# Luonic/semi-supervised_semantic_segmentation

Hardware: AMD Instinct MI355X
Metric: images/sec (UNet-R50 512x512 bs=16/GPU, mean-teacher + CowMix semi-supervised training step) (higher is better)
Workload: dtype bf16; 1 GPU; C2: UNet(ResNet-50 encoder, max_width=128, ConvT up) 512x512, semi-supervised mean-teacher + CowMix step (BCE sup loss w=0.5, consistency w=10, SGD m=0.9); global_batch=16, per_gpu_batch=16, image_size=512, parallelism=dp1

## Files before the change

include/ssseg.h:

```cpp
#ifndef SSSEG_H
#define SSSEG_H
#include <stdint.h>
#include <stddef.h>

#ifdef __cplusplus
extern "C" {
#endif

typedef struct ihipStream_t* ssseg_stream_t;

enum { SSSEG_F32 = 0, SSSEG_BF16 = 1, SSSEG_F16 = 2, SSSEG_F64 = 3  };
enum { SSSEG_OK = 0, SSSEG_EINVAL = -1, SSSEG_EUNSUPPORTED = -2, SSSEG_EWORKSPACE = -3, SSSEG_ECOMM = -4 };

const char* ssseg_version(void);


size_t ssseg_cowmix_workspace_bytes(int64_t B, int64_t H, int64_t W);

int ssseg_cowmix_mask(const float* noise, const float* sigma, const float* p, int64_t B, int64_t H,
                      int64_t W, float* mask_out, float* field_out, float* thr_out, void* workspace,
                      size_t workspace_bytes, ssseg_stream_t stream);

int ssseg_normal_f32(float* out, int64_t n, uint64_t seed, uint64_t offset, ssseg_stream_t stream);

// ... 285 lines not shown
  int32_t relu;
  float slope;
  double* stats;
  int64_t stats_ld;
  int64_t* stats_rows_host;
} ssseg_conv_epilogue;
int ssseg_conv_igemm_epi(const void* x, const void* w, void* y, const ssseg_conv_desc* desc_host, int dt, int dt_out,
                         const ssseg_conv_epilogue* epi, void* ws, size_t ws_bytes, ssseg_stream_t stream);
int ssseg_conv_igemm_epi_actmask(const void* x, const void* w, void* y, const ssseg_conv_desc* desc_host, int dt,
                                 int dt_out, const ssseg_conv_epilogue* epi, int act, float slope, void* ws,
                                 size_t ws_bytes, ssseg_stream_t stream);
int ssseg_conv_igemm_epi_join(const void* x, const void* w, void* y, const ssseg_conv_desc* desc_host, int dt,
                              int dt_out, const ssseg_conv_epilogue* epi, const void* mask, int64_t ldm, void* ws,
                              size_t ws_bytes, ssseg_stream_t stream);
typedef struct {
  const void* x2;
  int64_t c1;
  int64_t ldx2;
} ssseg_vcat;

int ssseg_conv_igemm_epi_vcat(const void* x, const ssseg_vcat* vc, const void* w, void* y,
                              const ssseg_conv_desc* desc_host, int dt, int dt_out, const ssseg_conv_epilogue* epi,
                              void* ws, size_t ws_bytes, ssseg_stream_t stream);
int ssseg_conv_igemm_epi_vsplit(const void* x, const void* w, void* y, const ssseg_vcat* ysplit,
                                const ssseg_conv_desc* desc_host, int dt, int dt_out, const ssseg_conv_epilogue* epi,
                                void* ws, size_t ws_bytes, ssseg_stream_t stream);
int ssseg_conv_igemm_phases(const void* x, void* y, const ssseg_conv_desc* desc_host, int dt, int dt_out,
                            const ssseg_conv_epilogue* epi, int64_t nphase, const int64_t* phase_geom,
                            const void* const* w, ssseg_stream_t stream);
size_t ssseg_conv_igemm_phases_workspace_bytes(const ssseg_conv_desc* desc_host, int64_t nphase, int dt);
int ssseg_conv_igemm_phases_ws(const void* x, void* y, const ssseg_conv_desc* desc_host, int dt, int dt_out,
                               const ssseg_conv_epilogue* epi, int64_t nphase, const int64_t* phase_geom,
                               const void* const* w, void* ws, size_t ws_bytes, ssseg_stream_t stream);

int ssseg_conv_stem_epi(const void* x, const void* w4, void* y, const ssseg_conv_desc* desc_host, int dt,
                        const ssseg_conv_epilogue* epi, ssseg_stream_t stream);
size_t ssseg_conv_igemm_workspace_bytes(const ssseg_conv_desc* desc_host, int dt);

int ssseg_set_knob(int id, int value);

int64_t ssseg_tune_table_export(unsigned long long* keys_host, int32_t* variants_host, int64_t cap);
int ssseg_tune_table_import(const unsigned long long* keys_host, const int32_t* variants_host, int64_t n,
                            int overwrite);

size_t ssseg_conv_wgrad_workspace_bytes(const ssseg_conv_desc* desc_host, int dt);
int ssseg_conv_wgrad(const void* x, const void* dy, float* dw, const ssseg_conv_desc* desc_host, int dt, int64_t c_real,
                     int64_t k_real, int layout, int accumulate, void* ws, size_t ws_bytes, ssseg_stream_t stream);

size_t ssseg_conv_wgrad2_workspace_bytes(const ssseg_conv_desc* desc_host, int64_t n2, int dt);
int ssseg_conv_wgrad2(const void* x, const void* dy, const void* x2, const void* dy2, int64_t n2, float* dw,
                      const ssseg_conv_desc* desc_host, int dt, int64_t c_real, int64_t k_real, int layout,
                      int accumulate, void* ws, size_t ws_bytes, ssseg_stream_t stream);

int ssseg_conv_wgrad_vcat(const void* x, const ssseg_vcat* vc, const void* dy, float* dw,
                          const ssseg_conv_desc* desc_host, int dt, int64_t c_real, int64_t k_real, int layout,
                          int accumulate, void* ws, size_t ws_bytes, ssseg_stream_t stream);
int ssseg_conv_wgrad2_vcat(const void* x, const ssseg_vcat* vc, const void* dy, const void* x2, const ssseg_vcat* vc2,
                           const void* dy2, int64_t n2, float* dw, const ssseg_conv_desc* desc_host, int dt,
                           int64_t c_real, int64_t k_real, int layout, int accumulate, void* ws, size_t ws_bytes,
                           ssseg_stream_t stream);

int ssseg_weight_pack(const float* src, void* dst, int64_t Kd, int64_t Kr, int64_t Cd, int64_t Rs, int64_t Ss,
                      int64_t Cp, int layout, int64_t r0, int64_t rstep, int64_t Rn, int64_t s0, int64_t sstep,
                      int64_t Sn, int dt, ssseg_stream_t stream);

typedef struct ssseg_pack_desc {
// ... 239 lines not shown
```

semi-supervised_semantic_segmentation_amd/csrc/conv.hip:

```cpp
#include <mutex>
#include <algorithm>
#include <unordered_map>
#include <vector>

#include "conv_kernels.h"

int g_knobs[17] = {0, -1, 0, 0, 0, 1, 0, 0, 0, 0, 100, 0, 0, 0, 0, 0, 0};
thread_local int t_dsplit = 1;

constexpr long long TICKET_POOL = 1 << 20;
__device__ unsigned g_ticket_pool[TICKET_POOL];

unsigned* ticket_slots(long long n) {
  static unsigned* const base = [] {
    void* p = nullptr;
    return hipGetSymbolAddress(&p, HIP_SYMBOL(g_ticket_pool)) == hipSuccess ? (unsigned*)p : nullptr;
  }();
  static std::mutex mu;
  static long long next = 0;
  if (!base || n <= 0 || n > TICKET_POOL / 16) return nullptr;
  std::lock_guard<std::mutex> lk(mu);
  if (next + n > TICKET_POOL) next = 0;
  unsigned* p = base + next;
  next += n;
// ... 184 lines not shown
static int heuristic_variant(const ConvGeom& g) {
  auto tiles = [&](int bm, int bn) { return ((g.M + bm - 1) / bm) * ((g.K + bn - 1) / bn); };
  if (g.KK <= 128) return 0;
  if (g.C % 64) return 5;
  if (g.K > 64) return tiles(256, 128) >= 128 ? 6 : (tiles(128, 128) >= 256 ? 8 : 5);
  return tiles(64, 64) < 512 ? 10 : 0;
}

static int dsplit_plan(const ConvGeom& g, int nph) {
  const int kn = g_knobs[14];
  if (kn < 0 || g.KK == 0) return 1;
  const int nk = (g.C % 64 == 0) ? g.R * g.S * (g.C / 64) : (g.KK + 63) / 64;
  if (kn > 0) return (kn == 2 || kn == 4 || kn == 8) && nk >= kn ? kn : 1;
  const long long t = (long long)nph * ((g.M + 127) / 128) * ((g.K + 63) / 64);
  if (t < 512 && nk >= 64) return (t < 128 && nk >= 128) ? 4 : 2;
  if (t < 256 && nk >= 8) {
    int S = 8;
    while (S > 1 && (t * S > 512 || nk < 4 * S)) S >>= 1;
    return S;
  }
  return 1;
}

template <typename T, typename TO>
int run_variant(int v, const void* x, const void* w, void* y, const ConvGeom& g, const Epi<TO>& ep, unsigned xb,
                unsigned wb, hipStream_t s, float* ws, const PhaseTab* ph = nullptr, const void* x2 = nullptr,
                unsigned x2b = 0) {
  t_pw_rows = -1;
  if (t_dsplit > 1 && (v == 0 || v >= 24)) return -1;
  if constexpr (sizeof(TO) == 2) {
    if (v != 0) return launch_glds_cfg<TO>(v, x, w, y, g, ep, xb, wb, s, ws, ph, x2, x2b);
  }
  if (x2) return -1;
  ws = nullptr;
  if (ph && ph->n > 1) {
    int bm = 0;
    long long rows = 0;
    for (int p = 0; p < ph->n; ++p) {
      ConvGeom gp = g;
      gp.py = ph->py[p];
      gp.px = ph->px[p];
      gp.ooy = ph->ooy[p];
      gp.oox = ph->oox[p];
      Epi<TO> ep2 = ep;
      if (ep.stats) ep2.stats = ep.stats + rows * 2 * ep.sld;
      bm = dispatch_regstaged<T, TO>(x, ph->w[p], y, gp, ep2, ws, s);
      if (bm <= 0) return bm;
      rows += (g.M + bm - 1) / bm;
    }
    return bm;
  }
  return dispatch_regstaged<T, TO>(x, w, y, g, ep, ws, s);
}

template <typename T, typename TO>
int tune_variant(const void* x, const void* w, void* y, const ConvGeom& g, const Epi<TO>& ep, unsigned xb,
                 unsigned wb, hipStream_t s, float* ws, const PhaseTab* ph, const void* x2, unsigned x2b,
                 bool* cache_it) {
  hipStreamCaptureStatus cap = hipStreamCaptureStatusNone;
  const int heur = x2 && heuristic_variant(g) == 0 ? 5 : heuristic_variant(g);
  *cache_it = true;
  if (hipStreamIsCapturing(s, &cap) != hipSuccess || cap != hipStreamCaptureStatusNone) {
    *cache_it = false;
    return heur;
  }
  hipEvent_t e0, e1;
// ... 84 lines not shown
        v = (g.C > g.ldx || S > 1) ? 14 : 0;
        if (x2 && v == 0) return -1;
      } else if ((g.C > g.ldx || S > 1) && (g_knobs[4] == 24 || g_knobs[4] == 28)) {
        v = 14;
      }
      int r = run_variant<T, TO>(v, x, w, y, g, ep, (unsigned)xb, (unsigned)wb, s, wsv, ph, x2, (unsigned)x2b);
      if (r == -1 && S > 1 && g_knobs[4] != 0)
        return run_variant<T, TO>(14, x, w, y, g, ep, (unsigned)xb, (unsigned)wb, s, wsv, ph, x2, (unsigned)x2b);
      if (r == -1 && g_knobs[4] != 0 && !x2 && g.C % 64 && g.C <= g.ldx)
        return run_variant<T, TO>(0, x, w, y, g, ep, 0, 0, s, nullptr, ph);
      if (r == -1 && ep.zmask) {
        int hv = heuristic_variant(g);
        if ((g.C > g.ldx || S > 1) && (hv == 0 || hv >= 24)) hv = 14;
        return run_variant<T, TO>(hv, x, w, y, g, ep, (unsigned)xb, (unsigned)wb, s, S > 1 ? wsv : nullptr, ph);
      }
      if (r == -1 && g_knobs[4] >= 24 && g_knobs[4] <= 28) {
        const int hv = x2 && heuristic_variant(g) == 0 ? 5 : heuristic_variant(g);
        return run_variant<T, TO>(hv, x, w, y, g, ep, (unsigned)xb, (unsigned)wb, s, nullptr, ph, x2, (unsigned)x2b);
      }
      if (r == -1 && g_knobs[4] == 0 && v != 0) {
        int hv = x2 && heuristic_variant(g) == 0 ? 5 : heuristic_variant(g);
        if ((g.C > g.ldx || S > 1) && (hv == 0 || hv >= 24)) hv = 14;
        if (hv != v)
          return run_variant<T, TO>(hv, x, w, y, g, ep, (unsigned)xb, (unsigned)wb, s, wsv, ph, x2, (unsigned)x2b);
      }
      return r;
    }
  }
  if (x2) return -1;
  if (g.C > g.ldx) return SSSEG_EUNSUPPORTED;
  return run_variant<T, TO>(0, x, w, y, g, ep, 0, 0, s, nullptr, ph);
}

bool geom_ok(const ConvGeom& g, int dt) {
  const int vec = (dt == SSSEG_F32 ? 4 : 8);
  if (g.C % vec || g.ldx % vec || g.ldw % vec) return false;
  if (g.N < 1 || g.OH < 1 || g.OW < 1 || g.K < 1 || g.C < 1) return false;
  if (g.M >= 0x7fffffffLL) return false;
  if (g.R < 0 || g.S < 0) return false;
  return true;
}

}

extern "C" int ssseg_set_knob(int id, int value) {
  if (id < 0 || id >= 17) return SSSEG_EINVAL;
  if (id == 6 && value) {
    std::lock_guard<std::mutex> lk(g_variant_mu);
    g_variant.clear();
    return 0;
  }
  g_knobs[id] = value;
  return 0;
}

extern "C" int64_t ssseg_tune_table_export(unsigned long long* keys_host, int32_t* variants_host, int64_t cap) {
  std::lock_guard<std::mutex> lk(g_variant_mu);
  if (cap > 0 && (!keys_host || !variants_host)) return SSSEG_EINVAL;
  std::vector<std::pair<unsigned long long, int>> rows(g_variant.begin(), g_variant.end());
  std::sort(rows.begin(), rows.end());
  const int64_t n = (int64_t)rows.size();
  for (int64_t i = 0; i < n && i < cap; ++i) {
    keys_host[i] = rows[i].first;
    variants_host[i] = rows[i].second;
  }
  return n;
// ... 250 lines not shown
    const int64_t* q = phase_geom + 4 * p;
    for (int k = 0; k < 4; ++k)
      if (q[k] < -0x40000000LL || q[k] > 0x40000000LL) return SSSEG_EINVAL;
    if (!w[p]) return SSSEG_EINVAL;
    ph.py[p] = (int)q[0];
    ph.px[p] = (int)q[1];
    ph.ooy[p] = (int)q[2];
    ph.oox[p] = (int)q[3];
    ph.w[p] = w[p];
  }
  g.py = ph.py[0];
  g.px = ph.px[0];
  g.ooy = ph.ooy[0];
  g.oox = ph.oox[0];
  hipStream_t s = (hipStream_t)stream;
  const size_t need = igemm_ws_bytes(g, dt, (int)nphase);
  float* wsf = (need > 0 && ws && ws_bytes >= need) ? (float*)ws : nullptr;
  int bm;
  if (dt == SSSEG_BF16) {
    const Epi<bf16_t> eb{e.scale, e.shift, (const bf16_t*)e.residual, (int)e.ldr, e.relu, (bf16_t*)e.aux, e.slope,
                         e.stats, (int)e.stats_ld};
    bm = dispatch_igemm<bf16_t, bf16_t>(x, w[0], y, g, eb, wsf, s, &ph);
  } else {
    const Epi<f16_t> eh{e.scale, e.shift, (const f16_t*)e.residual, (int)e.ldr, e.relu, (f16_t*)e.aux, e.slope,
                        e.stats, (int)e.stats_ld};
    bm = dispatch_igemm<f16_t, f16_t>(x, w[0], y, g, eh, wsf, s, &ph);
  }
  if (bm <= 0) return SSSEG_EUNSUPPORTED;
  if (e.stats_rows_host && e.stats) *e.stats_rows_host = nphase * ((g.M + bm - 1) / bm);
  SSSEG_LAUNCH_CHECK();
  return 0;
}

extern "C" int ssseg_conv_igemm_phases(const void* x, void* y, const ssseg_conv_desc* d, int dt, int dt_out,
                                       const ssseg_conv_epilogue* epi, int64_t nphase, const int64_t* phase_geom,
                                       const void* const* w, ssseg_stream_t stream) {
  return ssseg_conv_igemm_phases_ws(x, y, d, dt, dt_out, epi, nphase, phase_geom, w, nullptr, 0, stream);
}
```

semi-supervised_semantic_segmentation_amd/csrc/conv_kernels.h:

```cpp
#pragma once
#include <algorithm>
#include <type_traits>

#include "common.h"

typedef __bf16 bf16x8 __attribute__((ext_vector_type(8)));
typedef _Float16 f16x8 __attribute__((ext_vector_type(8)));

typedef short s16x4 __attribute__((ext_vector_type(4)));
typedef float f32x4 __attribute__((ext_vector_type(4)));

template <typename T16> struct M16;
template <> struct M16<bf16_t> {
  __device__ __forceinline__ static f32x4 mma(const bf16x8& a, const bf16x8& b, const f32x4& c) {
    return __builtin_amdgcn_mfma_f32_16x16x32_bf16(a, b, c, 0, 0, 0);
  }
};
template <> struct M16<f16_t> {
  __device__ __forceinline__ static f32x4 mma(const bf16x8& a, const bf16x8& b, const f32x4& c) {
    return __builtin_amdgcn_mfma_f32_16x16x32_f16(__builtin_bit_cast(f16x8, a), __builtin_bit_cast(f16x8, b), c, 0, 0,
                                                  0);
  }
};
typedef __attribute__((address_space(3))) s16x4 lds_s16x4;
// ... 161 lines not shown
    for (int e = 0; e < V; ++e) {
      s1[e] += __shfl_xor(s1[e], o, 64);
      s2[e] += __shfl_xor(s2[e], o, 64);
    }
  }
  lds_barrier();
  double* red = (double*)smem;
  const int w = threadIdx.x >> 6;
  if (holder)
#pragma unroll
    for (int e = 0; e < V; ++e) {
      red[(w * BN + cofs + e) * 2] = (double)s1[e];
      red[(w * BN + cofs + e) * 2 + 1] = (double)s2[e];
    }
  lds_barrier();
  for (int c = threadIdx.x; c < BN; c += NW * 64) {
    const int n = n0 + c;
    if (n >= sld || (dbg & 4)) continue;
    double a = 0.0, b = 0.0;
#pragma unroll
    for (int k = 0; k < NW; ++k) {
      a += red[(k * BN + c) * 2];
      b += red[(k * BN + c) * 2 + 1];
    }
    stats[(mtile * 2) * sld + n] = a;
    stats[(mtile * 2 + 1) * sld + n] = b;
  }
}

struct PhaseTab {
  int n;
  int py[4], px[4], ooy[4], oox[4];
  const void* w[4];
};

template <typename TO> struct Load4;
template <> struct Load4<float> {
  __device__ __forceinline__ static void ld(const float* p, float (&v)[4]) {
    const float4 q = *(const float4*)p;
    v[0] = q.x; v[1] = q.y; v[2] = q.z; v[3] = q.w;
  }
};
template <> struct Load4<f16_t> {
  __device__ __forceinline__ static void ld(const f16_t* p, float (&v)[4]) { H16::ld4(p, v); }
};
template <> struct Load4<bf16_t> {
  __device__ __forceinline__ static void ld(const bf16_t* p, float (&v)[4]) {
    const uint2 q = *(const uint2*)p;
    v[0] = __uint_as_float(q.x << 16); v[1] = __uint_as_float(q.x & 0xffff0000u);
    v[2] = __uint_as_float(q.y << 16); v[3] = __uint_as_float(q.y & 0xffff0000u);
  }
};

template <typename TO, int FM, int FN, bool ST = false, bool JOIN = false>
__device__ __forceinline__ void store_tile(const f32x4 (&acc)[FN][FM], long long mb, int nb, int lane,
                                           const ConvGeom& g, TO* __restrict__ y, const Epi<TO>& ep,
                                           double (*st1)[4] = nullptr, double (*st2)[4] = nullptr) {
  long long op[FM];
#pragma unroll
  for (int j = 0; j < FM; ++j) {
    const long long m = mb + j * 16 + (lane & 15);
    op[j] = -1;
    if (m < g.M) {
      op[j] = out_pixel(g, (int)m);
    }
  }
// ... 715 lines not shown
                                                                float* __restrict__ ws, unsigned* tix, PhaseTab ph,
                                                                const TO* __restrict__ x2, unsigned x2bytes) {
  constexpr int ROW = 128;
  constexpr bool VC = KM == 1, GK = KM == 2;
  constexpr int STAGE = (BM + BN) * ROW;
  constexpr int AI = BM / 8 / NW;
  constexpr int BI = BN / 8 / NW;
  constexpr int NL = AI + BI;
  constexpr int WTM = BM / WM, WTN = BN / WN, FM = WTM / 16, FN = WTN / 16;
  static_assert(WM * WN == NW && FM >= 1 && FN >= 1 && AI >= 1 && BI >= 1 && NS >= 1 && NS <= 4, "tile");
  constexpr int EPI = BM * (BN * 4 + 16);
  constexpr int SMEM = (NS == 1 && EPI > STAGE) ? EPI : NS * STAGE;
  __shared__ __attribute__((aligned(1024))) char smem[SMEM];

  const int t = threadIdx.x, lane = t & 63, wave = __builtin_amdgcn_readfirstlane(t >> 6);
  const int wm = wave / WN, wn = wave % WN;
  const int nnt = (g.K + BN - 1) / BN;
  const int lsp = 31 - __builtin_clz((unsigned)splits);
  const int bid = xcd_tile(blockIdx.x, gridDim.x);
  const int tile = bid >> lsp, slice = bid & (splits - 1);
  static_assert(BN == 64 || BN == 128 || BN == 256, "n-tile divisor magic");
  const int mt_ = fdiv(tile, BN == 64 ? g.mn64 : (BN == 128 ? g.mn128 : g.mn256),
                       BN == 64 ? g.sn64 : (BN == 128 ? g.sn128 : g.sn256));
  const long long m0 = (long long)mt_ * BM;
  const int n0 = (tile - mt_ * nnt) * BN;
  if (ph.n > 1) {
    const int p = blockIdx.y;
    g.py = ph.py[p];
    g.px = ph.px[p];
    g.ooy = ph.ooy[p];
    g.oox = ph.oox[p];
    w = (const TO*)ph.w[p];
    if (ep.stats) ep.stats += (long long)p * ((g.M + BM - 1) / BM) * 2 * ep.sld;
  }
  const int RS = g.R * g.S;
  const int cpt = g.C >> 6;
  const int nk_all = GK ? (g.KK + 63) >> 6 : RS * cpt;
  int kt0 = 0, nk = nk_all;
  if (splits > 1) {
    const int kper = (nk_all + splits - 1) / splits;
    kt0 = min(nk_all, slice * kper);
    nk = min(nk_all, kt0 + kper) - kt0;
  }
  const __amdgpu_buffer_rsrc_t xr = __builtin_amdgcn_make_buffer_rsrc((void*)x, (short)0, (int)xbytes, 0x00020000);
  const __amdgpu_buffer_rsrc_t wr = __builtin_amdgcn_make_buffer_rsrc((void*)w, (short)0, (int)wbytes, 0x00020000);
  __amdgpu_buffer_rsrc_t xr2 = xr;
  if constexpr (VC) xr2 = __builtin_amdgcn_make_buffer_rsrc((void*)x2, (short)0, (int)x2bytes, 0x00020000);

  const int c_even = (lane & 7) ^ (lane >> 4);
  int a_off[AI], a_iy[AI], a_ix[AI];
  int a_pix[VC ? AI : 1];
  int a_k[GK ? AI : 1];
#pragma unroll
  for (int ii = 0; ii < AI; ++ii) {
    const int inst = wave * AI + ii;
    const int ch = c_even ^ ((inst & 1) * 4);
    const long long m = m0 + 8 * inst + (lane >> 3);
    int pix = 0;
    if (m < g.M && g.aident) {
      a_iy[ii] = 0;
      a_ix[ii] = 0;
      pix = (int)m;
    } else if (m < g.M) {
      int img, oy, ox;
      decode_m(g, (int)m, img, oy, ox);
      a_iy[ii] = oy * g.sy + g.py;
// ... 376 lines not shown
```

semi-supervised_semantic_segmentation_amd/ssseg/native.py:

```python
import ctypes
import os
import re

import torch

_HERE = os.path.dirname(os.path.abspath(__file__))
LIB_PATH = os.environ.get('SSSEG_LIB_PATH') or os.path.join(_HERE, 'libssseg.so')
HEADER = os.path.join(_HERE, '..', '..', 'include', 'ssseg.h')

F32, BF16, F16, F64 = 0, 1, 2, 3
SSSEG_SUM, SSSEG_AVG = 0, 1
_ERRS = {-1: 'SSSEG_EINVAL', -2: 'SSSEG_EUNSUPPORTED', -3: 'SSSEG_EWORKSPACE', -4: 'SSSEG_ECOMM'}

vp, i64, i32, f32, f64, sz, u64 = (ctypes.c_void_p, ctypes.c_int64, ctypes.c_int, ctypes.c_float, ctypes.c_double,
                                   ctypes.c_size_t, ctypes.c_uint64)
I64P = ctypes.POINTER(ctypes.c_int64)

class CatPart(ctypes.Structure):
    _fields_ = [('src', vp), ('dst', vp), ('add', vp), ('ld', i64), ('c', i64)]


def cat_parts(rows):
    return (CatPart * len(rows))(*[CatPart(*r) for r in rows])

# ... 77 lines not shown
    'ssseg_dice_prob_bwd': (i32, [vp, i64, i64, i32, f32, vp, vp, vp, sz, vp]),
    'ssseg_binary_entropy_fwd': (i32, [vp, i64, vp, vp, sz, vp]),
    'ssseg_binary_entropy_bwd': (i32, [vp, i64, vp, vp, vp]),
    'ssseg_entropy_fwd': (i32, [vp, i64, i64, i64, vp, vp, sz, vp]),
    'ssseg_entropy_bwd': (i32, [vp, i64, i64, i64, vp, vp, vp]),
    'ssseg_bce_logits_red_fwd': (i32, [vp, vp, i64, i32, vp, vp, sz, vp]),
    'ssseg_bce_logits_red_bwd': (i32, [vp, vp, i64, i32, vp, vp, vp]),
    'ssseg_smooth_labels': (i32, [vp, vp, i64, f32, f32, vp]),
    'ssseg_uncertainty_workspace_bytes': (sz, [i64, i64, i64]),
    'ssseg_uncertainty_scores': (i32, [vp, i64, i64, i64, vp, vp, sz, vp]),
    'ssseg_kmeans_workspace_bytes': (sz, [i64, i64, i64]),
    'ssseg_kmeans_seed': (i32, [vp, i64, i64, i64, vp, vp, vp, vp, sz, vp]),
    'ssseg_kmeans_fit': (i32, [vp, i64, i64, i64, f64, i64, vp, vp, vp, vp, vp, sz, vp]),
    'ssseg_prob_onehot': (i32, [vp, i64, i64, vp, vp, vp]),
    'ssseg_seg_metrics': (i32, [vp, I64P, i64, i64, vp, I64P, i64, i64, i64, vp, vp, vp, vp]),
    'ssseg_seg_metrics_mc': (i32, [vp, I64P, i64, i64, vp, I64P, i32, i32, i64, i64, i64, i64, i64, vp, vp, vp, vp,
                                   vp]),
    'ssseg_prob_onehot_mc': (i32, [vp, i64, i64, i64, i32, vp, vp, vp]),
    'ssseg_ema_update': (i32, [vp, vp, i64, f64, vp]),
    'ssseg_scale_f32': (i32, [vp, i64, f32, vp]),
    'ssseg_axpby': (i32, [vp, f32, vp, f32, vp, i64, vp]),
    'ssseg_sigmoid_fwd': (i32, [vp, vp, i64, vp]),
    'ssseg_sigmoid_bwd': (i32, [vp, vp, vp, i64, vp]),
    'ssseg_sqnorm_accum': (i32, [vp, i64, vp, vp, sz, vp]),
    'ssseg_sgd_step': (i32, [vp, vp, vp, vp, i64, f32, f32, f32, f32, vp, i32, vp, vp]),
    'ssseg_optim_prepare': (i32, [vp, i32, f64, f64, f64, f64, f64, i64, f64, vp, vp, vp]),
    'ssseg_optim_step': (i32, [vp, vp, vp, vp, vp, vp, vp, i64, i32, i32, f64, f64, f64, f64, f64, f64, vp, vp]),
    'ssseg_amp_update': (i32, [vp, vp, f32, f32, i32, vp]),
    'ssseg_scale_by': (i32, [vp, vp, vp, i64, vp]),
    'ssseg_conv_igemm': (i32, [vp, vp, vp, vp, i32, i32, vp, i32, vp, sz, vp]),
    'ssseg_conv_igemm_phases': (i32, [vp, vp, vp, i32, i32, vp, i64, vp, vp, vp]),
    'ssseg_conv_igemm_phases_ws': (i32, [vp, vp, vp, i32, i32, vp, i64, vp, vp, vp, sz, vp]),
    'ssseg_conv_igemm_phases_workspace_bytes': (sz, [vp, i64, i32]),
    'ssseg_conv_stem_epi': (i32, [vp, vp, vp, vp, i32, vp, vp]),
    'ssseg_conv_igemm_epi': (i32, [vp, vp, vp, vp, i32, i32, vp, vp, sz, vp]),
    'ssseg_conv_igemm_epi_actmask': (i32, [vp, vp, vp, vp, i32, i32, vp, i32, f32, vp, sz, vp]),
    'ssseg_conv_igemm_epi_join': (i32, [vp, vp, vp, vp, i32, i32, vp, vp, i64, vp, sz, vp]),
    'ssseg_weight_pack_batch': (i32, [vp, i64, i32, vp]),
    'ssseg_param_step': (i32, [vp, vp, vp, vp, vp, i64, vp, f32, f32, f32, f32, vp, i32, vp, f64, i32, vp]),
    'ssseg_dwconv_fwd': (i32, [vp, vp, vp, vp, i32, vp, vp]),
    'ssseg_dwconv_dgrad': (i32, [vp, vp, vp, vp, i32, vp]),
    'ssseg_dwconv_wgrad_workspace_bytes': (sz, [vp, i32]),
    'ssseg_dwconv_wgrad': (i32, [vp, vp, vp, vp, i32, i64, i32, vp, sz, vp]),
    'ssseg_conv_igemm_workspace_bytes': (sz, [vp, i32]),
    'ssseg_set_knob': (i32, [i32, i32]),
    'ssseg_tune_table_export': (i64, [vp, vp, i64]),
    'ssseg_tune_table_import': (i32, [vp, vp, i64, i32]),
    'ssseg_conv_wgrad_workspace_bytes': (sz, [vp, i32]),
    'ssseg_conv_wgrad': (i32, [vp, vp, vp, vp, i32, i64, i64, i32, i32, vp, sz, vp]),
    'ssseg_conv_wgrad2_workspace_bytes': (sz, [vp, i64, i32]),
    'ssseg_conv_wgrad2': (i32, [vp, vp, vp, vp, i64, vp, vp, i32, i64, i64, i32, i32, vp, sz, vp]),
    'ssseg_conv_igemm_epi_vcat': (i32, [vp, vp, vp, vp, vp, i32, i32, vp, vp, sz, vp]),
    'ssseg_conv_igemm_epi_vsplit': (i32, [vp, vp, vp, vp, vp, i32, i32, vp, vp, sz, vp]),
    'ssseg_conv_wgrad_vcat': (i32, [vp, vp, vp, vp, vp, i32, i64, i64, i32, i32, vp, sz, vp]),
    'ssseg_conv_wgrad2_vcat': (i32, [vp, vp, vp, vp, vp, vp, i64, vp, vp, i32, i64, i64, i32, i32, vp, sz, vp]),
    'ssseg_weight_pack': (i32, [vp, vp, i64, i64, i64, i64, i64, i64, i32, i64, i64, i64, i64, i64, i64, i32, vp]),
    'ssseg_bn_workspace_bytes': (sz, [i64]),
    'ssseg_bn_stats': (i32, [vp, i64, i64, i64, i32, vp, vp, sz, vp]),
    'ssseg_bn_partials_finalize': (i32, [vp, i64, i64, vp, f64, f32, f32, vp, vp, vp, vp, vp, vp]),
    'ssseg_bn_gstat_finalize': (i32, [vp, i64, i64, vp, vp, vp, vp, vp, vp, vp, vp, vp]),
    'ssseg_bn_gstat_finalize_x': (i32, [vp, i64, i64, vp, vp, vp, vp, vp, i64, i64, i32, vp, vp, vp, vp, vp]),
    'ssseg_channel_sum_grad': (i32, [vp, i64, i64, i64, i32, vp, vp, vp, sz, vp]),
    'ssseg_bn_finalize': (i32, [vp, i64, f64, f32, f32, vp, vp, vp, vp, vp, vp]),
    'ssseg_bn_eval_params': (i32, [vp, vp, f32, i64, vp, vp, vp]),
    'ssseg_bn_fold': (i32, [vp, vp, vp, vp, vp, f32, i64, i64, vp, vp, vp, vp, vp]),
    'ssseg_bn_fold_batch': (i32, [vp, i64, vp]),
# ... 166 lines not shown
```

semi-supervised_semantic_segmentation_amd/ssseg/nn.py:

```python
import contextlib
import ctypes
import os

import torch
import torch.distributed as dist
import torch.nn as nn

from . import comm as _comm
from . import native as N

_CFG = {'act_mask': os.environ.get('SSSEG_ACT_MASK', '1') != '0',
        'grad_join': True, 'stem': os.environ.get('SSSEG_STEM', '1') != '0', 'phases': True, 'eval_bwd_y': True, 'dtype': torch.bfloat16, 'sync_bn': True,
        'fuse_stats': True, 'vcat': os.environ.get('SSSEG_VCAT', '1') != '0',
        'vpad': os.environ.get('SSSEG_VPAD', '1') != '0',
        'bn_gstat': os.environ.get('SSSEG_BN_GSTAT', '1') != '0',
        'bn_join': os.environ.get('SSSEG_BN_JOIN', '1') != '0'}


_QUANT = [None]


def set_bn_grad_stats(on):
    _CFG['bn_gstat'] = bool(on)


def set_bn_join(on):
    _CFG['bn_join'] = bool(on)


def _bn_join_on():
    return _CFG['bn_join'] and _CFG['bn_gstat'] and _CFG['act_mask']


def set_virtual_concat(on):
    _CFG['vcat'] = bool(on)


def set_eval_bwd_from_y(on):
    _CFG['eval_bwd_y'] = bool(on)


def set_phase_launch(on):
    _CFG['phases'] = bool(on)


def set_stem_kernel(on):
    _CFG['stem'] = bool(on)


def set_grad_join(on):
    _CFG['grad_join'] = bool(on)


def set_compute_dtype(dtype):
    assert dtype in (torch.bfloat16, torch.float16, torch.float32)
    _CFG['dtype'] = dtype


def compute_dtype():
    return _CFG['dtype']


def set_sync_bn(flag):
    _CFG['sync_bn'] = bool(flag)


_WGRAD = {'merge': os.environ.get('SSSEG_WGRAD_MERGE', '1') != '0', 'defer': False, 'pending': []}


def set_wgrad_merge(on):
    _WGRAD['merge'] = bool(on)


@contextlib.contextmanager
def defer_wgrad():
    if not _WGRAD['merge']:
# ... 292 lines not shown
def to_act_cat(xs):
    n = sum(int(x.shape[0]) for x in xs)
    _, c, h, w = xs[0].shape
    cp = rup(c, vec())
    y = new_act(n, cp, h, w, _CFG['dtype'], xs[0].device)
    off = 0
    for x in xs:
        if tuple(x.shape[1:]) != (c, h, w):
            raise ValueError('to_act_cat: batches of different image shapes')
        xc = x if x.is_contiguous() else x.contiguous()
        N.call('ssseg_nchw_to_nhwc', N.dev_ptr(xc, 'image'), N.dev_ptr(y) + off * cp * h * w * y.element_size(),
               int(x.shape[0]), c, h, w, cp, N.dt_code(xc), N.dt_code(y), N.stream())
        off += int(x.shape[0])
    return y


def _desc(**kw):
    d = N.ConvDesc()
    for k, v in kw.items():
        setattr(d, k, int(v))
    return d


def _phases(stride, pad, R, in_full, dil=1):
    assert dil == 1, 'strided transposed contraction with dilation is not supported'
    out = []
    for phi in range(stride):
        r0 = (phi + pad) % stride
        rn = 0 if r0 >= R else (R - r0 + stride - 1) // stride
        delta = (phi + pad - r0) // stride
        q = (in_full - phi + stride - 1) // stride
        out.append((phi, r0, rn, delta, max(q, 0)))
    return out


ACT_NONE, ACT_RELU, ACT_RELU6, ACT_LEAKY = 0, 1, 2, 3


def _act(a):
    if a is None or a is False:
        return ACT_NONE, 0.0
    if a is True:
        return ACT_RELU, 0.0
    if isinstance(a, tuple):
        if a[0] != 'leaky':
            raise ValueError(f'unknown activation {a!r}')
        return ACT_LEAKY, float(a[1])
    code = int(a)
    if code not in (ACT_NONE, ACT_RELU, ACT_RELU6):
        raise ValueError(f'unknown activation {a!r}')
    return code, 0.0


class GradHandoff:
    __slots__ = ('grad',)

    def __init__(self):
        self.grad = None

    def put(self, g):
        if self.grad is not None:
            raise RuntimeError('GradHandoff: gradient already pending')
        self.grad = g

    def take(self):
        g, self.grad = self.grad, None
# ... 536 lines not shown
            (scale, None, None, None) if scale is not None else None)
        cin, cout = self._dims()
        n, _, H, W = xshape
        (R, S), (sh, sw), (ph, pw), (dh, dw) = self.kernel_size, self.stride, self.padding, self.dilation
        OH, OW = gy.shape[2], gy.shape[3]
        dx = new_act(n, cin, H, W, _CFG['dtype'], gy.device)
        if residual is not None:
            _need_res(residual, dx)
            if self._ssseg_dw:
                raise NotImplementedError('ssseg.nn.Conv2d: fused input-gradient accumulation needs a dense conv')
        if self._ssseg_dw:
            d = self._dw_desc(n, H, W)
            with _Timed(2.0 * n * OH * OW * self.in_channels * R * S, 'dgrad', _tag(self, n, H, W)):
                N.call('ssseg_dwconv_dgrad', N.dev_ptr(gy), N.dev_ptr(self._dw_pack()), N.dev_ptr(dx), ctypes_ref(d),
                       N.dt_code(gy), N.stream())
            return dx
        timer = _Timed(_conv_flops(n, OH, OW, self.out_channels, self.in_channels, R, S), 'dgrad', _tag(self, n, H, W))
        ce = vpad(cout) if self._vpad_ok() else cout
        if sh == 1 and sw == 1:
            w = self._pack('dgrad', cin, self.in_channels, self.out_channels, ce, 1, R - 1, -1, R, S - 1, -1, S)
            d = _desc(N=n, H=OH, W=OW, C=ce, ldx=cout, OH=H, OW=W, K=cin, R=R, S=S, sy=1, sx=1, dy=dh, dx=dw,
                      py=ph - (R - 1) * dh, px=pw - (S - 1) * dw, outH=H, outW=W, osy=1, osx=1, ooy=0, oox=0,
                      ldy=cin, ldw=R * S * ce)
            with timer:
                if join is not None:
                    if self._igemm(gy, w, dx, d, N.dt_code(dx), fold=fold, join=join):
                        dx.__dict__['_ssseg_premasked'] = True
                    else:
                        self._igemm(gy, w, dx, d, N.dt_code(dx), fold=fold)
                else:
                    self._igemm(gy, w, dx, d, N.dt_code(dx), fold=fold, mask=mask, stats=stats)
            return dx
        timer.__enter__()
        for (phy, ry0, rny, dly, qy) in _phases(sh, ph, R, H, dh):
            for (phx, rx0, rnx, dlx, qx) in _phases(sw, pw, S, W, dw):
                if qy == 0 or qx == 0:
                    continue
                rr, ss = (rny, rnx) if rny * rnx > 0 else (0, 0)
                w = self._pack(('dgrad', phy, phx), cin, self.in_channels, self.out_channels, ce, 1, ry0, sh,
                               rny, rx0, sw, rnx) if rr else None
                d = _desc(N=n, H=OH, W=OW, C=ce, ldx=cout, OH=qy, OW=qx, K=cin, R=rr, S=ss, sy=1, sx=1, dy=-1,
                          dx=-1, py=dly, px=dlx, outH=H, outW=W, osy=sh, osx=sw, ooy=phy, oox=phx, ldy=cin,
                          ldw=max(rr * ss * ce, ce))
                self._igemm(gy, w, dx, d, N.dt_code(dx), fold=fold, mask=mask, stats=stats)
        timer.__exit__()
        return dx


    def _ssseg_dgrad_vsplit(self, gy, xshape, vc):
        cin, cout = self._dims()
        n, cp, H, W = xshape
        if (self._ssseg_dw or self.stride != (1, 1) or cp != vc.ca + vc.cb or cin != cp
                or _CFG['dtype'] not in (torch.bfloat16, torch.float16)):
            return None
        (R, S), (ph, pw), (dh, dw) = self.kernel_size, self.padding, self.dilation
        OH, OW = gy.shape[2], gy.shape[3]
        da = new_act(n, vc.ca, H, W, _CFG['dtype'], gy.device)
        db = new_act(n, vc.cb, H, W, _CFG['dtype'], gy.device)
        w = self._pack('dgrad', cin, self.in_channels, self.out_channels, cout, 1, R - 1, -1, R, S - 1, -1, S)
        d = _desc(N=n, H=OH, W=OW, C=cout, ldx=cout, OH=H, OW=W, K=cin, R=R, S=S, sy=1, sx=1, dy=dh, dx=dw,
                  py=ph - (R - 1) * dh, px=pw - (S - 1) * dw, outH=H, outW=W, osy=1, osx=1, ooy=0, oox=0,
                  ldy=vc.ca, ldw=R * S * cout)
        dref = ctypes_ref(d)
        nb = N.lib().ssseg_conv_igemm_workspace_bytes(dref, N.dt_code(gy))
        ws = N.workspace(nb, gy.device) if nb else None
        mask = vc.a if vc.mask_a else None
        ep = N.ConvEpilogue(None, None, N.dev_ptr(mask) if mask is not None else None, vc.ca if mask is not None else 0,
                            None, 0, 0.0, None, 0, None)
        split = N.VCat(N.dev_ptr(db), vc.ca, vc.cb)
        with _Timed(_conv_flops(n, OH, OW, self.out_channels, self.in_channels, R, S), 'dgrad', _tag(self, n, H, W)):
            ok = N.call_or_unsupported('ssseg_conv_igemm_epi_vsplit', N.dev_ptr(gy), N.dev_ptr(w), N.dev_ptr(da),
                                       ctypes_ref(split), dref, N.dt_code(gy), N.dt_code(gy), ctypes_ref(ep),
                                       N.dev_ptr(ws) if ws is not None else None, nb, N.stream())
        if not ok:
            return None
        if mask is not None:
            da.__dict__['_ssseg_premasked'] = True
        return da, db


# ... 1018 lines not shown
```

Baseline: 535.3 images/sec.

## Launch strided-conv dgrad phases with differing tap counts in one kernel

Adds a heterogeneous phase launch for strided convolution data-gradients. Sub-pixel phases with different filter tap extents now run in a single igemm launch that switches R/S, weights and divisors per phase, instead of one launch per phase. This is meant to cut launch overhead and tail underutilisation for the strided convs in backward. It adds per-phase geometry handling inside the kernel, and the old loop remains as a fallback when the plan is rejected.

```diff
diff --git a/include/ssseg.h b/include/ssseg.h
--- a/include/ssseg.h
+++ b/include/ssseg.h
@@ -341,6 +341,12 @@
 int ssseg_conv_igemm_phases_ws(const void* x, void* y, const ssseg_conv_desc* desc_host, int dt, int dt_out,
                                const ssseg_conv_epilogue* epi, int64_t nphase, const int64_t* phase_geom,
                                const void* const* w, void* ws, size_t ws_bytes, ssseg_stream_t stream);
+size_t ssseg_conv_igemm_dgrad_phases_workspace_bytes(const ssseg_conv_desc* desc_host, int64_t nphase,
+                                                     const int64_t* phase_geom, int dt);
+int ssseg_conv_igemm_dgrad_phases(const void* x, void* y, const ssseg_conv_desc* desc_host, int dt, int dt_out,
+                                  const ssseg_conv_epilogue* epi, int act, float slope, int64_t nphase,
+                                  const int64_t* phase_geom, const void* const* w, void* ws, size_t ws_bytes,
+                                  ssseg_stream_t stream);
 
 int ssseg_conv_stem_epi(const void* x, const void* w4, void* y, const ssseg_conv_desc* desc_host, int dt,
                         const ssseg_conv_epilogue* epi, ssseg_stream_t stream);
diff --git a/semi-supervised_semantic_segmentation_amd/csrc/conv.hip b/semi-supervised_semantic_segmentation_amd/csrc/conv.hip
--- a/semi-supervised_semantic_segmentation_amd/csrc/conv.hip
+++ b/semi-supervised_semantic_segmentation_amd/csrc/conv.hip
@@ -240,6 +240,7 @@
     if (v != 0) return launch_glds_cfg<TO>(v, x, w, y, g, ep, xb, wb, s, ws, ph, x2, x2b);
   }
   if (x2) return -1;
+  if (ph && ph->n > 1 && ph->het) return -1;
   ws = nullptr;
   if (ph && ph->n > 1) {
     int bm = 0;
@@ -390,6 +391,135 @@
   return run_variant<T, TO>(0, x, w, y, g, ep, 0, 0, s, nullptr, ph);
 }
 
+bool geom_ok(const ConvGeom& g, int dt);
+
+struct HetPlan {
+  PhaseTab ph;
+  ConvGeom g;
+  int S;
+  int hv;
+};
+
+static ConvGeom het_phase_geom(const ConvGeom& g, const PhaseTab& ph, int p) {
+  ConvGeom gp = g;
+  gp.R = ph.R[p];
+  gp.S = ph.S[p];
+  gp.py = ph.py[p];
+  gp.px = ph.px[p];
+  gp.ooy = ph.ooy[p];
+  gp.oox = ph.oox[p];
+  gp.KK = gp.R * gp.S * gp.C;
+  gp.ldw = gp.KK;
+  return gp;
+}
+
+static int het_plan(const ssseg_conv_desc* d, int64_t nphase, const int64_t* phase_geom, int dt, HetPlan& hp) {
+  if (!d || !phase_geom || nphase < 2 || nphase > 4) return SSSEG_EINVAL;
+  if (dt != SSSEG_BF16 && dt != SSSEG_F16) return SSSEG_EUNSUPPORTED;
+  int best = -1;
+  long long best_taps = 0;
+  for (int p = 0; p < (int)nphase; ++p) {
+    const int64_t* q = phase_geom + 6 * p;
+    for (int k = 0; k < 4; ++k)
+      if (q[k] < -0x40000000LL || q[k] > 0x40000000LL) return SSSEG_EINVAL;
+    if (q[4] < 0 || q[5] < 0 || q[4] > 64 || q[5] > 64 || ((q[4] == 0) != (q[5] == 0))) return SSSEG_EINVAL;
+    if (q[4] * q[5] > best_taps) {
+      best_taps = q[4] * q[5];
+      best = p;
+    }
+  }
+  if (best < 0) return SSSEG_EUNSUPPORTED;
+  ssseg_conv_desc dd = *d;
+  dd.R = phase_geom[6 * best + 4];
+  dd.S = phase_geom[6 * best + 5];
+  if (dd.C < 0 || dd.C > 0x7fffffff || dd.R * dd.S * dd.C > 0x7fffffffLL) return SSSEG_EINVAL;
+  dd.ldw = dd.R * dd.S * dd.C;
+  dd.py = phase_geom[6 * best];
+  dd.px = phase_geom[6 * best + 1];
+  dd.ooy = phase_geom[6 * best + 2];
+  dd.oox = phase_geom[6 * best + 3];
+  ConvGeom& g = hp.g;
+  if (!make_geom(&dd, g) || !geom_ok(g, dt)) return SSSEG_EINVAL;
+  if (g.sy != 1 || g.sx != 1) return SSSEG_EINVAL;
+  hp.ph = PhaseTab{(int)nphase, {0}, {0}, {0}, {0}, {nullptr}};
+  hp.ph.het = 1;
+  for (int p = 0; p < (int)nphase; ++p) {
+    const int64_t* q = phase_geom + 6 * p;
+    hp.ph.py[p] = (int)q[0];
+    hp.ph.px[p] = (int)q[1];
+    hp.ph.ooy[p] = (int)q[2];
+    hp.ph.oox[p] = (int)q[3];
+    hp.ph.R[p] = (int)q[4];
+    hp.ph.S[p] = (int)q[5];
+    fdiv_init(q[5] > 0 ? (int)q[5] : 1, hp.ph.mS[p], hp.ph.sS[p]);
+  }
+  const long long xb = (long long)g.N * g.H * g.W * g.ldx * 2;
+  if (g_knobs[3] != 0 || g.ldx % 8 || g.K <= 16 || xb >= 0x7fffffffLL) return SSSEG_EUNSUPPORTED;
+  hp.S = 0;
+  hp.hv = -1;
+  for (int p = 0; p < (int)nphase; ++p) {
+    if (hp.ph.R[p] == 0) continue;
+    const ConvGeom gp = het_phase_geom(g, hp.ph, p);
+    if ((long long)gp.K * gp.ldw * 2 >= 0x7fffffffLL) return SSSEG_EUNSUPPORTED;
+    const int S = dsplit_plan(gp, 1);
+    if (hp.S != 0 && S != hp.S) return SSSEG_EUNSUPPORTED;
+    hp.S = S;
+    int hv = heuristic_variant(gp);
+    if (gp.C > gp.ldx && (hv == 0 || hv == 24 || hv == 28)) hv = 14;
+    if (S > 1 && (hv == 0 || hv >= 24)) hv = 14;
+    hp.hv = hp.hv == -1 || hp.hv == hv ? hv : 0;
+  }
+  if (hp.hv < 0 || hp.hv >= 24) hp.hv = 0;
+  g.aident = g.H == g.OH && g.W == g.OW;
+  return 0;
+}
+
+static unsigned long long het_key(unsigned long long h, const PhaseTab& ph) {
+  h = (h ^ 0x9e3779b97f4a7c15ull) * 1099511628211ull;
+  for (int p = 0; p < ph.n; ++p) h = (h ^ (unsigned long long)(ph.R[p] * 65 + ph.S[p] + 1)) * 1099511628211ull;
+  return h;
+}
+
+template <typename TO>
+int dispatch_het(const void* x, void* y, const HetPlan& hp, const Epi<TO>& ep, float* ws, hipStream_t s) {
+  const ConvGeom& g = hp.g;
+  const unsigned xb = (unsigned)((long long)g.N * g.H * g.W * g.ldx * 2), wb = (unsigned)((long long)g.K * g.ldw * 2);
+  const PhaseTab* ph = &hp.ph;
+  const void* w = nullptr;
+  for (int p = 0; p < ph->n; ++p)
+    if (ph->R[p] && !w) w = ph->w[p];
+  DsplitScope scope(hp.S);
+  float* wsv = hp.S > 1 ? ws : nullptr;
+  if (hp.S > 1 && !wsv) return -1;
+  int v = g_knobs[4];
+  if (v == 11 || v >= 24) return -1;
+  if (v <= 0) {
+    const unsigned long long key = het_key(
+        geom_key(g, (int)sizeof(TO) * 8 + (ep.stats ? 4 : 0) + (ep.res ? 2 : 0) + (ep.scale ? 1 : 0) + 16 * hp.S +
+                        256 * ph->n + (ep.rmask ? (1 << 25) : 0) + (ep.gstat ? (1 << 26) : 0)),
+        *ph);
+    std::lock_guard<std::mutex> lk(g_variant_mu);
+    auto it = g_variant.find(key);
+    if (it != g_variant.end()) {
+      v = it->second;
+    } else if (!g_knobs[5]) {
+      v = hp.hv;
+      if (v == 0) return -1;
+      g_variant[key] = v;
+    } else {
+      bool cache_it = true;
+      v = tune_variant<TO, TO>(x, w, y, g, ep, xb, wb, s, wsv, ph, nullptr, 0, &cache_it);
+      if (!cache_it) v = hp.hv;
+      if (v == 0 || v >= 24) v = 14;
+      if (cache_it) g_variant[key] = v;
+    }
+  }
+  int r = run_variant<TO, TO>(v, x, w, y, g, ep, xb, wb, s, wsv, ph);
+  if (r == -1 && g_knobs[4] <= 0 && hp.hv > 0 && hp.hv != v)
+    r = run_variant<TO, TO>(hp.hv, x, w, y, g, ep, xb, wb, s, wsv, ph);
+  return r;
+}
+
 bool geom_ok(const ConvGeom& g, int dt) {
   const int vec = (dt == SSSEG_F32 ? 4 : 8);
   if (g.C % vec || g.ldx % vec || g.ldw % vec) return false;
@@ -706,6 +836,62 @@
   return 0;
 }
 
+extern "C" size_t ssseg_conv_igemm_dgrad_phases_workspace_bytes(const ssseg_conv_desc* d, int64_t nphase,
+                                                                const int64_t* phase_geom, int dt) {
+  HetPlan hp;
+  if (het_plan(d, nphase, phase_geom, dt, hp) != 0) return 0;
+  return dsplit_ws_bytes(hp.g, (int)nphase, hp.S);
+}
+
+extern "C" int ssseg_conv_igemm_dgrad_phases(const void* x, void* y, const ssseg_conv_desc* d, int dt, int dt_out,
+                                             const ssseg_conv_epilogue* epi, int act, float slope, int64_t nphase,
+                                             const int64_t* phase_geom, const void* const* w, void* ws,
+                                             size_t ws_bytes, ssseg_stream_t stream) {
+  if (!x || !y || !w || dt != dt_out) return SSSEG_EINVAL;
+  if (act != 0 && act != SSSEG_ACT_RELU && act != SSSEG_ACT_LEAKY) return SSSEG_EINVAL;
+  HetPlan hp;
+  const int rc = het_plan(d, nphase, phase_geom, dt, hp);
+  if (rc != 0) return rc;
+  const ConvGeom& g = hp.g;
+  for (int p = 0; p < (int)nphase; ++p) {
+    if (hp.ph.R[p] && !w[p]) return SSSEG_EINVAL;
+    hp.ph.w[p] = hp.ph.R[p] ? w[p] : nullptr;
+  }
+  const ssseg_conv_epilogue none = {nullptr, nullptr, nullptr, 0, nullptr, 0, 0.f, nullptr, 0, nullptr};
+  const ssseg_conv_epilogue& e = epi ? *epi : none;
+  if (e.residual && (e.ldr < g.K || e.ldr > 0x7fffffff)) return SSSEG_EINVAL;
+  if (e.stats && (!e.stats_rows_host || e.stats_ld < 1 || e.stats_ld > g.K)) return SSSEG_EINVAL;
+  const bool gst = act != 0 && e.stats != nullptr;
+  if (e.stats && !gst && (e.scale || e.residual || e.relu || e.aux)) return SSSEG_EINVAL;
+  if (e.relu < 0 || e.relu > SSSEG_ACT_LEAKY) return SSSEG_EINVAL;
+  if (act && (!e.residual || e.aux || e.relu || e.shift)) return SSSEG_EINVAL;
+  if (e.stats_rows_host) *e.stats_rows_host = 0;
+  if (g.M == 0) return 0;
+  hipStream_t s = (hipStream_t)stream;
+  const size_t need = dsplit_ws_bytes(g, (int)nphase, hp.S);
+  float* wsf = (need > 0 && ws && ws_bytes >= need) ? (float*)ws : nullptr;
+  int bm;
+  if (dt == SSSEG_BF16) {
+    Epi<bf16_t> eb{e.scale, e.shift, (const bf16_t*)e.residual, (int)e.ldr, e.relu, (bf16_t*)e.aux, e.slope,
+                   e.stats, (int)e.stats_ld};
+    eb.rmask = act;
+    eb.rslope = slope;
+    eb.gstat = gst ? 1 : 0;
+    bm = dispatch_het<bf16_t>(x, y, hp, eb, wsf, s);
+  } else {
+    Epi<f16_t> eh{e.scale, e.shift, (const f16_t*)e.residual, (int)e.ldr, e.relu, (f16_t*)e.aux, e.slope,
+                  e.stats, (int)e.stats_ld};
+    eh.rmask = act;
+    eh.rslope = slope;
+    eh.gstat = gst ? 1 : 0;
+    bm = dispatch_het<f16_t>(x, y, hp, eh, wsf, s);
+  }
+  if (bm <= 0) return SSSEG_EUNSUPPORTED;
+  if (e.stats_rows_host && e.stats) *e.stats_rows_host = nphase * ((g.M + bm - 1) / bm);
+  SSSEG_LAUNCH_CHECK();
+  return 0;
+}
+
 extern "C" int ssseg_conv_igemm_phases(const void* x, void* y, const ssseg_conv_desc* d, int dt, int dt_out,
                                        const ssseg_conv_epilogue* epi, int64_t nphase, const int64_t* phase_geom,
                                        const void* const* w, ssseg_stream_t stream) {
diff --git a/semi-supervised_semantic_segmentation_amd/csrc/conv_kernels.h b/semi-supervised_semantic_segmentation_amd/csrc/conv_kernels.h
--- a/semi-supervised_semantic_segmentation_amd/csrc/conv_kernels.h
+++ b/semi-supervised_semantic_segmentation_amd/csrc/conv_kernels.h
@@ -217,6 +217,10 @@
   int n;
   int py[4], px[4], ooy[4], oox[4];
   const void* w[4];
+  int het;
+  int R[4], S[4];
+  unsigned mS[4];
+  int sS[4];
 };
 
 template <typename TO> struct Load4;
@@ -998,6 +1002,16 @@
     g.oox = ph.oox[p];
     w = (const TO*)ph.w[p];
     if (ep.stats) ep.stats += (long long)p * ((g.M + BM - 1) / BM) * 2 * ep.sld;
+    if (ph.het) {
+      g.R = ph.R[p];
+      g.S = ph.S[p];
+      g.mS = ph.mS[p];
+      g.sS = ph.sS[p];
+      g.KK = g.R * g.S * g.C;
+      g.ldw = g.KK;
+      wbytes = (unsigned)g.K * (unsigned)g.KK * 2u;
+      g.aident = g.aident && g.R == 1 && g.S == 1 && g.py == 0 && g.px == 0;
+    }
   }
   const int RS = g.R * g.S;
   const int cpt = g.C >> 6;
diff --git a/semi-supervised_semantic_segmentation_amd/ssseg/native.py b/semi-supervised_semantic_segmentation_amd/ssseg/native.py
--- a/semi-supervised_semantic_segmentation_amd/ssseg/native.py
+++ b/semi-supervised_semantic_segmentation_amd/ssseg/native.py
@@ -133,6 +133,8 @@
     'ssseg_conv_igemm_phases': (i32, [vp, vp, vp, i32, i32, vp, i64, vp, vp, vp]),
     'ssseg_conv_igemm_phases_ws': (i32, [vp, vp, vp, i32, i32, vp, i64, vp, vp, vp, sz, vp]),
     'ssseg_conv_igemm_phases_workspace_bytes': (sz, [vp, i64, i32]),
+    'ssseg_conv_igemm_dgrad_phases': (i32, [vp, vp, vp, i32, i32, vp, i32, f32, i64, vp, vp, vp, sz, vp]),
+    'ssseg_conv_igemm_dgrad_phases_workspace_bytes': (sz, [vp, i64, vp, i32]),
     'ssseg_conv_stem_epi': (i32, [vp, vp, vp, vp, i32, vp, vp]),
     'ssseg_conv_igemm_epi': (i32, [vp, vp, vp, vp, i32, i32, vp, vp, sz, vp]),
     'ssseg_conv_igemm_epi_actmask': (i32, [vp, vp, vp, vp, i32, i32, vp, i32, f32, vp, sz, vp]),
diff --git a/semi-supervised_semantic_segmentation_amd/ssseg/nn.py b/semi-supervised_semantic_segmentation_amd/ssseg/nn.py
--- a/semi-supervised_semantic_segmentation_amd/ssseg/nn.py
+++ b/semi-supervised_semantic_segmentation_amd/ssseg/nn.py
@@ -14,7 +14,8 @@
         'fuse_stats': True, 'vcat': os.environ.get('SSSEG_VCAT', '1') != '0',
         'vpad': os.environ.get('SSSEG_VPAD', '1') != '0',
         'bn_gstat': os.environ.get('SSSEG_BN_GSTAT', '1') != '0',
-        'bn_join': os.environ.get('SSSEG_BN_JOIN', '1') != '0'}
+        'bn_join': os.environ.get('SSSEG_BN_JOIN', '1') != '0',
+        'dgrad_phases': os.environ.get('SSSEG_DGRAD_PHASES', '1') != '0'}
 
 
 _QUANT = [None]
@@ -42,6 +43,10 @@
 
 def set_phase_launch(on):
     _CFG['phases'] = bool(on)
+
+
+def set_dgrad_phase_launch(on):
+    _CFG['dgrad_phases'] = bool(on)
 
 
 def set_stem_kernel(on):
@@ -400,6 +405,39 @@
         q = (in_full - phi + stride - 1) // stride
         out.append((phi, r0, rn, delta, max(q, 0)))
     return out
+
+
+def dgrad_phase_table(kernel, stride, padding, in_hw):
+    (R, S), (sh, sw), (ph, pw), (H, W) = kernel, stride, padding, in_hw
+    tab = []
+    for (phy, ry0, rny, dly, qy) in _phases(sh, ph, R, H):
+        for (phx, rx0, rnx, dlx, qx) in _phases(sw, pw, S, W):
+            if qy == 0 or qx == 0:
+                continue
+            tab.append(dict(phy=phy, phx=phx, qy=qy, qx=qx, ry0=ry0, rx0=rx0, rny=rny, rnx=rnx, dly=dly, dlx=dlx,
+                            taps=(rny, rnx) if rny * rnx > 0 else (0, 0)))
+    return tab
+
+
+def check_phase_table(tab, kernel, stride, in_hw):
+    (R, S), (sh, sw), (H, W) = kernel, stride, in_hw
+    taps, pix = {}, {}
+    for t in tab:
+        rr, ss = t['taps']
+        if (rr, ss) != ((t['rny'], t['rnx']) if t['rny'] * t['rnx'] > 0 else (0, 0)):
+            raise ValueError('phase table: packed tap extents differ from the phase\'s taps')
+        for j in range(rr):
+            for i in range(ss):
+                key = (t['ry0'] + sh * j, t['rx0'] + sw * i)
+                taps[key] = taps.get(key, 0) + 1
+        for y in range(t['qy']):
+            for x in range(t['qx']):
+                key = (t['phy'] + sh * y, t['phx'] + sw * x)
+                pix[key] = pix.get(key, 0) + 1
+    if taps != {(r, s): 1 for r in range(R) for s in range(S)}:
+        raise ValueError('phase table: the phases\' taps do not partition the filter')
+    if pix != {(y, x): 1 for y in range(H) for x in range(W)}:
+        raise ValueError('phase table: the phases\' sub-grids do not cover every input pixel exactly once')
 
 
 ACT_NONE, ACT_RELU, ACT_RELU6, ACT_LEAKY = 0, 1, 2, 3
@@ -1002,6 +1040,10 @@
                     self._igemm(gy, w, dx, d, N.dt_code(dx), fold=fold, mask=mask, stats=stats)
             return dx
         timer.__enter__()
+        if (_CFG['dgrad_phases'] and (dh, dw) == (1, 1) and _CFG['dtype'] in (torch.bfloat16, torch.float16)
+                and self._dgrad_phases(gy, dx, (n, H, W, OH, OW, cin, cout, ce), fold, mask, stats)):
+            timer.__exit__()
+            return dx
         for (phy, ry0, rny, dly, qy) in _phases(sh, ph, R, H, dh):
             for (phx, rx0, rnx, dlx, qx) in _phases(sw, pw, S, W, dw):
                 if qy == 0 or qx == 0:
@@ -1016,6 +1058,44 @@
         timer.__exit__()
         return dx
 
+
+    def _dgrad_phases(self, gy, dx, dims, fold, mask, stats):
+        import ctypes
+        n, H, W, OH, OW, cin, cout, ce = dims
+        sh, sw = self.stride
+        tab = dgrad_phase_table(self.kernel_size, self.stride, self.padding, (H, W))
+        if not (2 <= len(tab) <= 4) or len({(t['qy'], t['qx']) for t in tab}) != 1 or _vcat_of(gy) is not None:
+            return False
+        if not any(t['taps'][0] for t in tab):
+            return False
+        ws = [self._pack(('dgrad', t['phy'], t['phx']), cin, self.in_channels, self.out_channels, ce, 1, t['ry0'], sh,
+                         t['rny'], t['rx0'], sw, t['rnx']) if t['taps'][0] else None for t in tab]
+        d = _desc(N=n, H=OH, W=OW, C=ce, ldx=cout, OH=tab[0]['qy'], OW=tab[0]['qx'], K=cin, R=0, S=0, sy=1, sx=1,
+                  dy=-1, dx=-1, py=0, px=0, outH=H, outW=W, osy=sh, osx=sw, ooy=0, oox=0, ldy=cin, ldw=ce)
+        geo = (ctypes.c_int64 * (6 * len(tab)))(*[v for t in tab for v in (t['dly'], t['dlx'], t['phy'], t['phx'],
+                                                                           t['taps'][0], t['taps'][1])])
+        wp = (ctypes.c_void_p * len(tab))(*[N.dev_ptr(w) if w is not None else None for w in ws])
+        scale, shift, res, aux = fold if fold is not None else (None, None, None, None)
+        if mask is not None:
+            res = mask[0]
+        sf = stats.launch_fields() if stats is not None else (None, 0, None)
+        ep = N.ConvEpilogue(N.dev_ptr(scale) if scale is not None else None,
+                            N.dev_ptr(shift) if shift is not None else None,
+                            N.dev_ptr(res) if res is not None else None, res.shape[1] if res is not None else 0,
+                            N.dev_ptr(aux) if aux is not None else None, 0, 0.0, *sf)
+        dref = ctypes_ref(d)
+        nb = N.lib().ssseg_conv_igemm_dgrad_phases_workspace_bytes(dref, len(tab), ctypes.addressof(geo),
+                                                                   N.dt_code(gy))
+        scratch = N.workspace(nb, gy.device) if nb else None
+        if not N.call_or_unsupported(
+                'ssseg_conv_igemm_dgrad_phases', N.dev_ptr(gy), N.dev_ptr(dx), dref, N.dt_code(gy), N.dt_code(dx),
+                ctypes_ref(ep), int(mask[1]) if mask is not None else 0, float(mask[2]) if mask is not None else 0.0,
+                len(tab), ctypes.addressof(geo), ctypes.addressof(wp),
+                N.dev_ptr(scratch) if scratch is not None else None, nb, N.stream()):
+            return False
+        if stats is not None:
+            stats.commit()
+        return True
 
     def _ssseg_dgrad_vsplit(self, gy, xshape, vc):
         cin, cout = self._dims()
```

Measured after the change: 536.8 images/sec (median of 6 runs). About the same (+0.3%).
